# aghasemzadeh/OpenMPL

Measured on AMD Instinct MI355X. Metric: poses/sec (V=4, J=17, batch=1024 per GPU) fp32, higher is better.
Workload: dtype f32; 1 GPU; Human3.6M config: V=4 J=17 batch=1024 fp32, CHOSEN flag set, depth 12, DIM 32, heads 8; global_batch=1024, parallelism=single GPU

## Files before the change

openmpl_amd/csrc/spt_packed.hip:

```cpp
#include "spt_pack.hpp"
#include "spt_stage.hpp"

namespace mpl {

constexpr int ATS = 36;
constexpr int HS = 68;
constexpr int KV_F = SJ * SH * SEQ * 4;
constexpr int SPT3_RING_BYTES = (ROWS * XS + 2 * KV_F + ROWS * ATS) * 4;
constexpr int SPT3_LDS_BYTES = 160 * 1024;
constexpr int SPT3_HID_OFF = 3072;
constexpr int SPT3_Q_OFF = 20480;
static_assert(SPT3_HID_OFF + ROWS * HS <= 2 * KV_F + ROWS * ATS, "HID does not fit its alias");
static_assert((SPT3_HID_OFF + ROWS * HS - 2 * KV_F) * 4 <= SPT3_Q_OFF, "HID reaches into the staged qkv weights");
static_assert(SPT3_Q_OFF + 12 * 1024 <= ROWS * ATS * 4, "staged qkv weights do not fit behind HID in ATT");
static_assert(SPT3_RING_BYTES + 8 * 1024 + 2 * SPT3_NPAR * 4 <= SPT3_LDS_BYTES, "spare LDS too small");

typedef float f32x2 __attribute__((ext_vector_type(2)));

__device__ inline float spt_window_scale(float v) {
    if (!(v > 0.f) || !(v < 3.0e38f)) return 1.0f;
    int e;
    (void)frexpf(32768.0f / v, &e);
    e = e - 1 < -100 ? -100 : (e - 1 > 100 ? 100 : e - 1);
    return ldexpf(1.0f, e);
}

__global__ __launch_bounds__(256) void spt_pack_kernel(const float* __restrict__ qkv_w, const float* __restrict__ qkv_b,
                                                        const float* __restrict__ ln1_w, const float* __restrict__ ln1_b,
                                                        const float* __restrict__ proj_w, const float* __restrict__ proj_b,
                                                        const float* __restrict__ fc1_w, const float* __restrict__ fc1_b,
                                                        const float* __restrict__ ln2_w, const float* __restrict__ ln2_b,
                                                        const float* __restrict__ fc2_w, const float* __restrict__ fc2_b,
                                                        char* __restrict__ dst, int fold_q) {
    __shared__ float Wf[8192];
    __shared__ float cn[SPT_NCOL], sw[SPT_NCOL], bnd[SPT_NCOL], scal[2];
    const int tid = threadIdx.x;
    for (int i = tid; i < 8192; i += 256) {
        float w;
        if (i < 3072) w = qkv_w[i] * ln1_w[i & 31];
        else if (i < 4096) w = proj_w[i - 3072];
        else if (i < 6144) w = fc1_w[i - 4096] * ln2_w[i & 31];
        else w = fc2_w[i - 6144];
        Wf[i] = w;
    }
    __syncthreads();
    if (tid < SPT_NCOL) {
        const int n = tid;
        const float *wr, *raw, *beta = nullptr;
        int K = 32;
        float bias;
        if (n < 96) { wr = Wf + n * 32; raw = qkv_w + n * 32; beta = ln1_b; bias = qkv_b[n]; }
        else if (n < 128) { wr = Wf + 3072 + (n - 96) * 32; raw = proj_w + (n - 96) * 32; bias = proj_b[n - 96]; }
        else if (n < 192) { wr = Wf + 4096 + (n - 128) * 32; raw = fc1_w + (n - 128) * 32; beta = ln2_b; bias = fc1_b[n - 128]; }
        else { wr = Wf + 6144 + (n - 192) * 64; raw = fc2_w + (n - 192) * 64; bias = fc2_b[n - 192]; K = 64; }
        float amax = 0.f;
        double ss = 0.0, c = (double)bias;
        for (int k = 0; k < K; ++k) {
            amax = fmaxf(amax, fabsf(wr[k]));
            ss += (double)wr[k] * (double)wr[k];
            if (beta) c += (double)raw[k] * (double)beta[k];
        }
        float s = 1.0f;
        if (amax > 0.f && amax < 3.0e38f) {
            int e;
            (void)frexpf(amax, &e);
            e = 14 - e;
            e = e < -100 ? -100 : (e > 100 ? 100 : e);
            s = ldexpf(1.0f, e);
        }
        cn[n] = (float)c;
        sw[n] = s;
        bnd[n] = beta ? (float)(sqrt(32.0) * sqrt(ss)) + fabsf((float)c) : 0.f;
    }
    __syncthreads();
    if (tid == 0) {
        float batt = 0.f, bhid = 0.f;
        for (int n = 64; n < 96; ++n) batt = fmaxf(batt, bnd[n]);
        for (int n = SPT_C_FC1; n < SPT_C_FC2; ++n) bhid = fmaxf(bhid, bnd[n]);
        scal[0] = spt_window_scale(batt);
        scal[1] = spt_window_scale(bhid);
    }
    __syncthreads();
    float* vec = reinterpret_cast<float*>(dst + SPT_PACK_VEC);
    if (tid < SPT_NCOL) {
        const int n = tid;
        float c = cn[n], sc;
        if (n < 96) sc = 1.0f / (SPT_SA * sw[n]);
        else if (n < 128) sc = 1.0f / (scal[0] * sw[n]);
        else if (n < 192) sc = 1.0f / (SPT_SA * sw[n]);
        else sc = 1.0f / (scal[1] * sw[n]);
        if (n < 32 && fold_q) { c *= SPT_QS; sc *= SPT_QS; }
        vec[n] = c;
        vec[SPT_NCOL + n] = sc;
    }
    if (tid < 8) vec[2 * SPT_NCOL + tid] = tid == 0 ? scal[0] : (tid == 1 ? 0.5f * scal[1] : 0.f);
    sf16x8* frag = reinterpret_cast<sf16x8*>(dst);
    for (int idx = tid; idx < 16 * 64; idx += 256) {
        const int lane = idx & 63, u = idx >> 6, li = lane & 15, kq = lane >> 4;
        const float* src;
        int n;
        if (u < 6) { n = 16 * u + li; src = Wf + n * 32 + 8 * kq; }
        else if (u < 8) { n = 16 * (u - 6) + li; src = Wf + 3072 + n * 32 + 8 * kq; n += SPT_C_PROJ; }
        else if (u < 12) { n = 16 * (u - 8) + li; src = Wf + 4096 + n * 32 + 8 * kq; n += SPT_C_FC1; }
        else { n = 16 * ((u - 12) >> 1) + li; src = Wf + 6144 + n * 64 + 32 * ((u - 12) & 1) + 8 * kq; n += SPT_C_FC2; }
        float x[8];
#pragma unroll
        for (int j = 0; j < 8; ++j) x[j] = src[j] * sw[n];
        sf16x8 hi, lo;
        spt_split2(x, hi, lo);
        frag[(size_t)(u * 2) * 64 + lane] = hi;
        frag[(size_t)(u * 2 + 1) * 64 + lane] = lo;
    }
}

int launch_spt_pack(const mpl_block_weights* bw_host, unsigned short* dst, int fold_q, hipStream_t s) {
    const mpl_block_weights* b = bw_host;
    if (!b || !dst || !b->qkv_w || !b->proj_w || !b->fc1_w || !b->fc2_w || !b->qkv_b || !b->proj_b || !b->fc1_b || !b->fc2_b ||
        !b->ln1_w || !b->ln1_b || !b->ln2_w || !b->ln2_b)
        return MPL_E_INVALID;
    ProfScope prof(MPL_K_PACK, s);
    hipLaunchKernelGGL(spt_pack_kernel, dim3(1), dim3(256), 0, s, b->qkv_w, b->qkv_b, b->ln1_w, b->ln1_b, b->proj_w, b->proj_b, b->fc1_w,
                       b->fc1_b, b->ln2_w, b->ln2_b, b->fc2_w, b->fc2_b, reinterpret_cast<char*>(dst), fold_q);
    return hip_check_launch();
}

size_t spt_pack_bytes() { return SPT_PACK_BYTES; }

template <int SS>
__global__ __launch_bounds__(NTHR, 1) void spt3_kernel(const SptParams p) {
    constexpr int RLIVE = SJ * SS;
    constexpr int MTS = (RLIVE + 15) / 16;
    constexpr int NT = (MTS + 3) / 4;
    extern __shared__ __attribute__((aligned(16))) float smem[];
    float* X = smem;
    float* Kb = smem + ROWS * XS;
    float* Vb = Kb + KV_F;
    float* ATT = Vb + KV_F;
    float* HID = Kb + SPT3_HID_OFF;
    char* S_W = reinterpret_cast<char*>(ATT + ROWS * ATS);
    float* S_PAR = reinterpret_cast<float*>(S_W + 8 * 1024);
    char* R_F1 = reinterpret_cast<char*>(Kb);
    char* R_Q = reinterpret_cast<char*>(ATT) + SPT3_Q_OFF;

    const int tid = threadIdx.x, lane = tid & 63;
    const int wave = __builtin_amdgcn_readfirstlane(tid >> 6);
    const int li = lane & 15, kq = lane >> 4;
    auto phase_sync = [&]() {
        asm volatile("s_waitcnt vmcnt(0)" ::: "memory");
        __syncthreads();
    };
    const int hg = wave & 1, part = wave >> 1;
    const int view = blockIdx.x % p.V;
    const int b0 = (blockIdx.x / p.V) * SS;
    const int sl = li % SS;
    const mpl_spt_set set = p.sets[(p.flags & MPL_F_MULTI_SPT) ? view : 0];
    const float* pose = p.poses[view];
    const float* ray = p.rays[view];
    const float* cen = p.centers[view];

    auto stage_w = [&](char* dst, const unsigned short* pack, int byte_off, int n_pieces) {
        const unsigned l0 = (unsigned)(uintptr_t)(__attribute__((address_space(3))) char*)dst;
        for (int i = wave; i < n_pieces; i += NWAVE)
            ::mpl::dma16(reinterpret_cast<const float*>(reinterpret_cast<const char*>(pack) + byte_off + i * 1024) + lane * 4,
                         l0 + (unsigned)(i * 1024));
    };
    auto load_par = [&](const mpl_block_weights& b) -> float4 {
        if (tid >= SPT3_NPAR / 4) return float4{0.f, 0.f, 0.f, 0.f};
        return ld4(G(reinterpret_cast<const float*>(reinterpret_cast<const char*>(b.qkv_w3) + SPT_PACK_VEC)) + 4 * tid);
    };
    auto store_par = [&](int app_of, const float4& v) {
        if (tid < SPT3_NPAR / 4) st4(S_PAR + (app_of & 1) * SPT3_NPAR + 4 * tid, v);
    };
    mpl_block_weights bw;
    if (p.n_apps > 0) {
        bw = set.blocks[p.sched[0] & 0x7f];
        stage_w(R_Q, bw.qkv_w3, SPT_PACK_QKV, 12);
    }
    const float4 par0 = p.n_apps > 0 ? load_par(bw) : float4{0.f, 0.f, 0.f, 0.f};
    spt_embed<true, SS>(p, set, X, tid, b0, pose, ray, cen, SS, MTS * 16);
    store_par(0, par0);
    phase_sync();

    auto load_w = [&](const char* region, int unit, sf16x8 (&w)[2]) { spt_load_unit(region, unit, lane, w); };
    auto ln_frag = [&](int m, sf16x8& ah, sf16x8& al) {
        const float* xr = X + (m * 16 + li) * XS + 8 * kq;
        spt_ln_split(::mpl::ld4(xr), ::mpl::ld4(xr + 4), ah, al);
    };
    auto raw_frag = [&](const float* rowp, sf16x8& ah, sf16x8& al) {
        const float4 x0 = ::mpl::ld4(rowp), x1 = ::mpl::ld4(rowp + 4);
        const float y[8] = {x0.x, x0.y, x0.z, x0.w, x1.x, x1.y, x1.z, x1.w};
        spt_split2(y, ah, al);
    };

    for (int app = 0; app < p.n_apps; ++app) {
        const bool weighted = (p.sched[app] & 0x80) != 0;
        bw = set.blocks[p.sched[app] & 0x7f];
        const unsigned short* pack = bw.qkv_w3;
        const float* par = S_PAR + (app & 1) * SPT3_NPAR;
        stage_w(S_W, pack, SPT_PACK_PROJ, 4);
        {
            sf16x8 wq[3][2];
            float4 bq[3], sq[3];
#pragma unroll
            for (int c = 0; c < 3; ++c) {
                load_w(R_Q, 2 * c + hg, wq[c]);
                bq[c] = ::mpl::ld4(par + SPT_C_QKV + 32 * c + 16 * hg + 4 * kq);
                sq[c] = ::mpl::ld4(par + SPT_NCOL + SPT_C_QKV + 32 * c + 16 * hg + 4 * kq);
            }
            float4 q[NT];
#pragma unroll
            for (int t = 0; t < NT; ++t) {
                q[t] = float4{0.f, 0.f, 0.f, 0.f};
                if (part + 4 * t < MTS && !(p.abl & 8)) {
                    const int m = part + 4 * t;
                    const int j = (16 * m + li) / SS;
                    const bool live = 16 * m + li < RLIVE;
                    sf16x8 ah, al;
                    ln_frag(m, ah, al);
                    const f32x4 z = {0.f, 0.f, 0.f, 0.f};
                    const f32x4 cq = mfma3(wq[0], ah, al, z), ck = mfma3(wq[1], ah, al, z), cv = mfma3(wq[2], ah, al, z);
                    q[t] = float4{fmaf(cq[0], sq[0].x, bq[0].x), fmaf(cq[1], sq[0].y, bq[0].y), fmaf(cq[2], sq[0].z, bq[0].z),
                                  fmaf(cq[3], sq[0].w, bq[0].w)};
                    const int h = 4 * hg + kq;
                    const float kx = fmaf(ck[0], sq[1].x, bq[1].x), ky = fmaf(ck[1], sq[1].y, bq[1].y);
                    const float kz = fmaf(ck[2], sq[1].z, bq[1].z), kw = fmaf(ck[3], sq[1].w, bq[1].w);
                    if (live && j < SJ - 1) {
                        float* kp = Kb + ((((j >> 1) * 2) * SH + h) * SS + sl) * 4 + (j & 1);
                        kp[0] = kx;
                        kp[2] = ky;
                        kp[SH * SS * 4] = kz;
                        kp[SH * SS * 4 + 2] = kw;
                    } else if (live) {
                        st4(Kb + (SJ - 1) * SH * SS * 4 + (h * SS + sl) * 4, float4{kx, ky, kz, kw});
                    }
                    if (live)
                        st4(Vb + ((j * SH + h) * SS + sl) * 4, float4{fmaf(cv[0], sq[2].x, bq[2].x), fmaf(cv[1], sq[2].y, bq[2].y),
                                                                       fmaf(cv[2], sq[2].z, bq[2].z), fmaf(cv[3], sq[2].w, bq[2].w)});
                }
            }
            phase_sync();
            if (!(p.abl & 1)) {
                const int h = 4 * hg + kq;
                float sc[NT][SJ];
#pragma unroll
                for (int jp = 0; jp < SJ / 2; ++jp) {
                    const float4 k01 = ::mpl::ld4(Kb + (((jp * 2) * SH + h) * SS + sl) * 4);
                    const float4 k23 = ::mpl::ld4(Kb + (((jp * 2 + 1) * SH + h) * SS + sl) * 4);
                    const f32x2 kx = {k01.x, k01.y}, ky = {k01.z, k01.w}, kz = {k23.x, k23.y}, kw = {k23.z, k23.w};
#pragma unroll
                    for (int t = 0; t < NT; ++t) {
                        const f32x2 qx = {q[t].x, q[t].x}, qy = {q[t].y, q[t].y}, qz = {q[t].z, q[t].z}, qw = {q[t].w, q[t].w};
                        f32x2 s2 = qx * kx;
                        s2 = __builtin_elementwise_fma(qy, ky, s2);
                        s2 = __builtin_elementwise_fma(qz, kz, s2);
                        s2 = __builtin_elementwise_fma(qw, kw, s2);
                        sc[t][2 * jp] = s2[0];
                        sc[t][2 * jp + 1] = s2[1];
                    }
                }
                {
                    const float4 k = ::mpl::ld4(Kb + (SJ - 1) * SH * SS * 4 + (h * SS + sl) * 4);
#pragma unroll
                    for (int t = 0; t < NT; ++t)
                        sc[t][SJ - 1] = fmaf(q[t].w, k.w, fmaf(q[t].z, k.z, fmaf(q[t].y, k.y, q[t].x * k.x)));
                }
                const float s_att = par[2 * SPT_NCOL];
                float inv[NT];
#pragma unroll
                for (int t = 0; t < NT; ++t) {
                    float mx = sc[t][0];
#pragma unroll
                    for (int j = 1; j < SJ; ++j) mx = fmaxf(mx, sc[t][j]);
                    float l = 0.f;
#pragma unroll
                    for (int j = 0; j < SJ; ++j) {
                        sc[t][j] = __builtin_amdgcn_exp2f(sc[t][j] - mx);
                        l += sc[t][j];
                    }
                    inv[t] = __builtin_amdgcn_rcpf(l) * s_att;
                    if (weighted) {
                        const int b = b0 + sl, r = 16 * (part + 4 * t) + li;
                        inv[t] *= (b < p.B && r < RLIVE) ? pose[((size_t)b * SJ + r / SS) * 3 + 2] : 0.f;
                    }
                }
                float4 o[NT];
#pragma unroll
                for (int t = 0; t < NT; ++t) o[t] = float4{0.f, 0.f, 0.f, 0.f};
#pragma unroll
                for (int j = 0; j < SJ; ++j) {
                    const float4 v = ::mpl::ld4(Vb + ((j * SH + h) * SS + sl) * 4);
#pragma unroll
                    for (int t = 0; t < NT; ++t) {
                        const float pj = sc[t][j];
                        o[t].x = fmaf(pj, v.x, o[t].x);
                        o[t].y = fmaf(pj, v.y, o[t].y);
                        o[t].z = fmaf(pj, v.z, o[t].z);
                        o[t].w = fmaf(pj, v.w, o[t].w);
                    }
                }
#pragma unroll
                for (int t = 0; t < NT; ++t) {
                    o[t] = float4{o[t].x * inv[t], o[t].y * inv[t], o[t].z * inv[t], o[t].w * inv[t]};
                    if (weighted) {
                        const float big = fmaxf(fmaxf(fabsf(o[t].x), fabsf(o[t].y)), fmaxf(fabsf(o[t].z), fabsf(o[t].w)));
                        if (!(big <= 65000.f)) {
                            const float qn = __builtin_nanf("");
                            o[t] = float4{qn, qn, qn, qn};
                            if (p.err_host) __hip_atomic_fetch_or(p.err_host, 2u, __ATOMIC_RELAXED, __HIP_MEMORY_SCOPE_SYSTEM);
                        }
                    }
                }
#pragma unroll
                for (int t = 0; t < NT; ++t)
                    if (part + 4 * t < MTS) st4(ATT + ((part + 4 * t) * 16 + li) * ATS + 4 * h, o[t]);
            }
        }
        phase_sync();
        {
            stage_w(R_F1, pack, SPT_PACK_FC1, 8);
            sf16x8 wp[2][2];
            float4 bp[2], sp[2];
#pragma unroll
            for (int n = 0; n < 2; ++n) {
                load_w(S_W, n, wp[n]);
                bp[n] = ::mpl::ld4(par + SPT_C_PROJ + 16 * n + 4 * kq);
                sp[n] = ::mpl::ld4(par + SPT_NCOL + SPT_C_PROJ + 16 * n + 4 * kq);
            }
            const int lo = (MTS * 2 * wave) / NWAVE, hi = (MTS * 2 * (wave + 1)) / NWAVE;
            for (int m = lo >> 1; m <= ((hi - 1) >> 1) && !(p.abl & 32); ++m) {
                sf16x8 ah, al;
                raw_frag(ATT + (m * 16 + li) * ATS + 8 * kq, ah, al);
#pragma unroll
                for (int n = 0; n < 2; ++n) {
                    const int u = 2 * m + n;
                    if (u < lo || u >= hi) continue;
                    const f32x4 c = mfma3(wp[n], ah, al, f32x4{0.f, 0.f, 0.f, 0.f});
                    float* xd = X + (m * 16 + li) * XS + 16 * n + 4 * kq;
                    const float4 x = ::mpl::ld4(xd);
                    st4(xd, float4{x.x + fmaf(c[0], sp[n].x, bp[n].x), x.y + fmaf(c[1], sp[n].y, bp[n].y),
                                   x.z + fmaf(c[2], sp[n].z, bp[n].z), x.w + fmaf(c[3], sp[n].w, bp[n].w)});
                }
            }
        }
        phase_sync();
        {
            stage_w(S_W, pack, SPT_PACK_FC2, 8);
            sf16x8 w1[4][2];
            float4 b1[4], s1[4];
#pragma unroll
            for (int n = 0; n < 4; ++n) {
                load_w(R_F1, n, w1[n]);
                b1[n] = ::mpl::ld4(par + SPT_C_FC1 + 16 * n + 4 * kq);
                s1[n] = ::mpl::ld4(par + SPT_NCOL + SPT_C_FC1 + 16 * n + 4 * kq);
            }
            const float hs = par[2 * SPT_NCOL + 1];
            const int lo = (MTS * 4 * wave) / NWAVE, hi = (MTS * 4 * (wave + 1)) / NWAVE;
            for (int m = lo >> 2; m <= ((hi - 1) >> 2) && !(p.abl & 64); ++m) {
                sf16x8 ah, al;
                ln_frag(m, ah, al);
#pragma unroll
                for (int n = 0; n < 4; ++n) {
                    const int u = 4 * m + n;
                    if (u < lo || u >= hi) continue;
                    const f32x4 c = mfma3(w1[n], ah, al, f32x4{0.f, 0.f, 0.f, 0.f});
                    st4(HID + (m * 16 + li) * HS + 16 * n + 4 * kq,
                        float4{gelu_as_scaled(fmaf(c[0], s1[n].x, b1[n].x), hs), gelu_as_scaled(fmaf(c[1], s1[n].y, b1[n].y), hs),
                               gelu_as_scaled(fmaf(c[2], s1[n].z, b1[n].z), hs), gelu_as_scaled(fmaf(c[3], s1[n].w, b1[n].w), hs)});
                }
            }
        }
        phase_sync();
        {
            float4 parn = float4{0.f, 0.f, 0.f, 0.f};
            if (app + 1 < p.n_apps) {
                const mpl_block_weights bn = set.blocks[p.sched[app + 1] & 0x7f];
                stage_w(R_Q, bn.qkv_w3, SPT_PACK_QKV, 12);
                parn = load_par(bn);
            }
            sf16x8 w2[2][2][2];
            float4 b2[2], s2[2];
#pragma unroll
            for (int n = 0; n < 2; ++n) {
                load_w(S_W, 2 * n, w2[n][0]);
                load_w(S_W, 2 * n + 1, w2[n][1]);
                b2[n] = ::mpl::ld4(par + SPT_C_FC2 + 16 * n + 4 * kq);
                s2[n] = ::mpl::ld4(par + SPT_NCOL + SPT_C_FC2 + 16 * n + 4 * kq);
            }
            const int lo = (MTS * 2 * wave) / NWAVE, hi = (MTS * 2 * (wave + 1)) / NWAVE;
            for (int m = lo >> 1; m <= ((hi - 1) >> 1) && !(p.abl & 128); ++m) {
                sf16x8 ah0, al0, ah1, al1;
                raw_frag(HID + (m * 16 + li) * HS + 8 * kq, ah0, al0);
                raw_frag(HID + (m * 16 + li) * HS + 32 + 8 * kq, ah1, al1);
#pragma unroll
                for (int n = 0; n < 2; ++n) {
                    const int u = 2 * m + n;
                    if (u < lo || u >= hi) continue;
                    f32x4 c = mfma3(w2[n][0], ah0, al0, f32x4{0.f, 0.f, 0.f, 0.f});
                    c = mfma3(w2[n][1], ah1, al1, c);
                    float* xd = X + (m * 16 + li) * XS + 16 * n + 4 * kq;
                    const float4 x = ::mpl::ld4(xd);
                    st4(xd, float4{x.x + fmaf(c[0], s2[n].x, b2[n].x), x.y + fmaf(c[1], s2[n].y, b2[n].y),
                                   x.z + fmaf(c[2], s2[n].z, b2[n].z), x.w + fmaf(c[3], s2[n].w, b2[n].w)});
                }
            }
            if (app + 1 < p.n_apps) store_par(app + 1, parn);
        }
        phase_sync();
    }
    spt_epilogue<true, SS>(p, X, tid, view, b0, pose, ray, cen, SS, MTS * 16);
}

template <int SS>
static int launch_spt3(const SptParams& p, int grid, hipStream_t s) {
    if (int rc = kernel_lds_once<spt3_kernel<SS>>(SPT3_LDS_BYTES)) return rc;
    hipLaunchKernelGGL(spt3_kernel<SS>, dim3(grid), dim3(NTHR), SPT3_LDS_BYTES, s, p);
    return hip_check_launch();
}

int launch_spt_packed(const SptParams& p, int ss, int grid, hipStream_t s) {
    switch (ss) {
        case 1: return launch_spt3<1>(p, grid, s);
        case 2: return launch_spt3<2>(p, grid, s);
        case 4: return launch_spt3<4>(p, grid, s);
        case 8: return launch_spt3<8>(p, grid, s);
        case 16: return launch_spt3<16>(p, grid, s);
        default: return MPL_E_INVALID;
    }
}

}
```

openmpl_amd/csrc/spt_stage.hpp:

```cpp
#pragma once
#include "common.hpp"

namespace mpl {

constexpr int SJ = 17;
constexpr int SD = 32;
constexpr int SH = 8;
constexpr int SEQ = 16;
constexpr int ROWS = SEQ * SJ;
constexpr int XS = 36;
constexpr int NTHR = 512;
constexpr int NWAVE = NTHR / 64;
constexpr int SPT_SMALL_SPW = 8;

struct SptParams {
    const float* poses[MPL_MAX_VIEWS];
    const float* rays[MPL_MAX_VIEWS];
    const float* centers[MPL_MAX_VIEWS];
    const mpl_spt_set* sets;
    const float *snorm_w, *snorm_b;
    const float *pos3d_embed, *pos3d_view, *pos3d_lin_w, *pos3d_lin_b;
    const float *ray_w, *ray_b, *cfpt_w, *cfpt_b;
    float* xs;
    int B, V, in_ch, n_apps;
    unsigned flags;
    int c3;
    int spw;
    int abl;
    unsigned* err_host;
    unsigned char sched[MPL_MAX_APPS];
};

int launch_spt_native(const SptParams& p, int form, int grid, hipStream_t s);
int launch_spt_packed(const SptParams& p, int ss, int grid, hipStream_t s);

typedef const __attribute__((address_space(1))) float* gfp;
__device__ __forceinline__ gfp G(const float* p) { return (gfp)p; }
__device__ __forceinline__ float4 ld4(gfp p) {
    typedef float v4 __attribute__((ext_vector_type(4)));
    const v4 t = *reinterpret_cast<const __attribute__((address_space(1))) v4*>(p);
    return make_float4(t.x, t.y, t.z, t.w);
}

template <bool TM, int SS = SEQ>
__device__ __forceinline__ void row_to_sj(int r, int& sq, int& j) {
    if (TM) { j = r / SS; sq = r % SS; }
    else { sq = r / SJ; j = r - sq * SJ; }
}

template <bool TM, int SS = SEQ>
__device__ __forceinline__ void spt_embed(const SptParams& p, const mpl_spt_set& set, float* X, int tid, int b0,
                                          const float* pose, const float* ray, const float* cen, int nseq = SEQ, int nrows = ROWS) {
    for (int idx = tid; idx < nrows * SD; idx += NTHR) {
        const int r = idx >> 5, c = idx & 31;
        int sq, j;
        row_to_sj<TM, SS>(r, sq, j);
        const int b = b0 + sq;
        float x = 0.f;
        if (b < p.B && sq < nseq && j < SJ) {
            const float* in = pose + ((size_t)b * SJ + j) * 3;
            const float* we = set.embed_w + c * p.in_ch;
            x = set.embed_b[c] + we[0] * in[0] + we[1] * in[1];
            if (p.in_ch == 3) x += we[2] * in[2];
            if (p.flags & MPL_F_CONF_ADD) x += set.conf_w[c] * in[2] + set.conf_b[c];
            if (p.flags & MPL_F_CONF_MULT) x *= set.conf_w[c] * in[2] + set.conf_b[c];
            x += set.pos_embed[j * SD + c];
            if (p.flags & MPL_F_POS3D_SPATIAL) {
                if (p.flags & MPL_F_POS3D_LEARN) {
                    x += p.pos3d_embed[j * p.c3 + c];
                } else {
                    const float* rr = ray + ((size_t)b * SJ + j) * 3;
                    const float* cc = cen + (size_t)b * 3;
                    const float vx = rr[0] - cc[0], vy = rr[1] - cc[1], vz = rr[2] - cc[2];
                    const float nrm = fmaxf(sqrtf(vx * vx + vy * vy + vz * vz), 1e-12f);
                    const float* wl = p.pos3d_lin_w + c * 3;
                    x += p.pos3d_lin_b[c] + wl[0] * (vx / nrm) + wl[1] * (vy / nrm) + wl[2] * (vz / nrm);
                }
            }
        }
        X[r * XS + c] = x;
    }
}

template <bool TM, int SS = SEQ>
__device__ __forceinline__ void spt_epilogue(const SptParams& p, const float* X, int tid, int view, int b0, const float* pose,
                                             const float* ray, const float* cen, int nseq = SEQ, int nrows = ROWS) {
    const bool to_rays = (p.flags & MPL_F_POS3D_TO_RAYS) && (p.flags & MPL_F_RAYS_TOKEN);
    const bool ray_tok = !(p.flags & MPL_F_POS3D_TO_RAYS) && (p.flags & MPL_F_RAYS_TOKEN);
    const int cw = to_rays ? 2 * SD : SD;
    const int Df = SJ * SD * ((p.flags & MPL_F_RAYS_TOKEN) ? 2 : 1);
    for (int r = tid; r < nrows; r += NTHR) {
        int sq, j;
        row_to_sj<TM, SS>(r, sq, j);
        const int b = b0 + sq;
        if (b >= p.B || sq >= nseq || j >= SJ) continue;
        const float* xr = X + r * XS;
        float v[SD];
        float s = 0.f;
#pragma unroll
        for (int c = 0; c < SD; c += 4) {
            const float4 t = ld4(xr + c);
            v[c] = t.x; v[c + 1] = t.y; v[c + 2] = t.z; v[c + 3] = t.w;
            s += (t.x + t.y) + (t.z + t.w);
        }
        const float mean = s * (1.0f / 32.0f);
        float ss = 0.f;
#pragma unroll
        for (int c = 0; c < SD; ++c) {
            v[c] -= mean;
            ss = fmaf(v[c], v[c], ss);
        }
        const float rstd = 1.0f / sqrtf(ss * (1.0f / 32.0f) + 1e-6f);
        const float conf = pose[((size_t)b * SJ + j) * 3 + 2];
        float dx = 0.f, dy = 0.f, dz = 0.f, nx = 0.f, ny = 0.f, nz = 0.f;
        const bool need_dir = (p.flags & MPL_F_RAYS_TOKEN) ||
                              (!(p.flags & MPL_F_POS3D_SPATIAL) && !(p.flags & MPL_F_POS3D_LEARN));
        if (need_dir) {
            const float* rr = ray + ((size_t)b * SJ + j) * 3;
            const float* cc = cen + (size_t)b * 3;
            dx = rr[0] - cc[0]; dy = rr[1] - cc[1]; dz = rr[2] - cc[2];
            const float nrm = fmaxf(sqrtf(dx * dx + dy * dy + dz * dz), 1e-12f);
            nx = dx / nrm; ny = dy / nrm; nz = dz / nrm;
        }
        auto pos3d = [=](int c) -> float {
            if (p.flags & MPL_F_POS3D_SPATIAL) return p.pos3d_view[j * p.c3 + c];
            if (p.flags & MPL_F_POS3D_LEARN) return p.pos3d_embed[j * p.c3 + c];
            const float* wl = p.pos3d_lin_w + c * 3;
            return p.pos3d_lin_b[c] + wl[0] * nx + wl[1] * ny + wl[2] * nz;
        };
        auto ray_emb = [=](int c) -> float {
            const float* wr = p.ray_w + c * 3;
            return p.ray_b[c] + wr[0] * dx + wr[1] * dy + wr[2] * dz;
        };
        float* orow = p.xs + ((size_t)b * p.V + view) * Df;
        float* o1 = orow + j * cw;
#pragma unroll
        for (int c = 0; c < SD; c += 4) {
            float t[4];
#pragma unroll
            for (int q = 0; q < 4; ++q) {
                float y = v[c + q] * rstd * p.snorm_w[c + q] + p.snorm_b[c + q];
                if (p.flags & MPL_F_CONF_IN_FPT) y += p.cfpt_w[c + q] * conf + p.cfpt_b[c + q];
                t[q] = y + pos3d(c + q);
            }
            st4(o1 + c, float4{t[0], t[1], t[2], t[3]});
        }
        if (to_rays) {
#pragma unroll
            for (int c = 0; c < SD; c += 4) {
                float t[4];
#pragma unroll
                for (int q = 0; q < 4; ++q) t[q] = ray_emb(c + q) + pos3d(SD + c + q);
                st4(o1 + SD + c, float4{t[0], t[1], t[2], t[3]});
            }
        } else if (ray_tok) {
            float* o2 = orow + (SJ + j) * SD;
#pragma unroll
            for (int c = 0; c < SD; c += 4) st4(o2 + c, float4{ray_emb(c), ray_emb(c + 1), ray_emb(c + 2), ray_emb(c + 3)});
        }
    }
}

}
```

Before: 830,000 poses/s.

## Templatize spt3 kernel on wave count and split attention into full and tail tiles

The spt3 kernel now takes the wave count as a template parameter and launches 16 waves for larger sequence tiles, 8 otherwise, spreading row tiles across more waves. Attention is restructured into a lambda run separately for full tiles and one ragged tail tile, which avoids per-tile bounds checks. Scores and outputs are held as packed f32x2 so packed FMA can be used. The aim is more parallelism per block and less divergence and register pressure in attention, at the cost of more threads sharing the same LDS and barriers.

Measured after the change: 831,500 poses/s (median of 3 runs). No clear change (+0.2%).

```diff
diff --git a/openmpl_amd/csrc/spt_packed.hip b/openmpl_amd/csrc/spt_packed.hip
--- a/openmpl_amd/csrc/spt_packed.hip
+++ b/openmpl_amd/csrc/spt_packed.hip
@@ -126,11 +126,13 @@
 
 size_t spt_pack_bytes() { return SPT_PACK_BYTES; }
 
-template <int SS>
-__global__ __launch_bounds__(NTHR, 1) void spt3_kernel(const SptParams p) {
+template <int SS, int NW>
+__global__ __launch_bounds__(NW * 64, 1) void spt3_kernel(const SptParams p) {
     constexpr int RLIVE = SJ * SS;
     constexpr int MTS = (RLIVE + 15) / 16;
-    constexpr int NT = (MTS + 3) / 4;
+    constexpr int NWQ = NW / 2;
+    constexpr int NT = (MTS + NWQ - 1) / NWQ;
+    constexpr int NTF = MTS / NWQ;
     extern __shared__ __attribute__((aligned(16))) float smem[];
     float* X = smem;
     float* Kb = smem + ROWS * XS;
@@ -142,17 +144,25 @@
     char* R_F1 = reinterpret_cast<char*>(Kb);
     char* R_Q = reinterpret_cast<char*>(ATT) + SPT3_Q_OFF;
 
-    const int tid = threadIdx.x, lane = tid & 63;
+    const int tid = threadIdx.x;
+    int lane = tid & 63;
     const int wave = __builtin_amdgcn_readfirstlane(tid >> 6);
-    const int li = lane & 15, kq = lane >> 4;
+    int li = lane & 15, kq = lane >> 4;
     auto phase_sync = [&]() {
         asm volatile("s_waitcnt vmcnt(0)" ::: "memory");
         __syncthreads();
     };
     const int hg = wave & 1, part = wave >> 1;
+    auto has_tile = [&](int t) { return t < NTF || part + NWQ * t < MTS; };
     const int view = blockIdx.x % p.V;
     const int b0 = (blockIdx.x / p.V) * SS;
-    const int sl = li % SS;
+    int sl = li % SS;
+    auto relane = [&]() {
+        asm volatile("" : "+v"(lane));
+        li = lane & 15;
+        kq = lane >> 4;
+        sl = li % SS;
+    };
     const mpl_spt_set set = p.sets[(p.flags & MPL_F_MULTI_SPT) ? view : 0];
     const float* pose = p.poses[view];
     const float* ray = p.rays[view];
@@ -160,7 +170,7 @@
 
     auto stage_w = [&](char* dst, const unsigned short* pack, int byte_off, int n_pieces) {
         const unsigned l0 = (unsigned)(uintptr_t)(__attribute__((address_space(3))) char*)dst;
-        for (int i = wave; i < n_pieces; i += NWAVE)
+        for (int i = wave; i < n_pieces; i += NW)
             ::mpl::dma16(reinterpret_cast<const float*>(reinterpret_cast<const char*>(pack) + byte_off + i * 1024) + lane * 4,
                          l0 + (unsigned)(i * 1024));
     };
@@ -177,7 +187,7 @@
         stage_w(R_Q, bw.qkv_w3, SPT_PACK_QKV, 12);
     }
     const float4 par0 = p.n_apps > 0 ? load_par(bw) : float4{0.f, 0.f, 0.f, 0.f};
-    spt_embed<true, SS>(p, set, X, tid, b0, pose, ray, cen, SS, MTS * 16);
+    spt_embed<true, SS, NW * 64>(p, set, X, tid, b0, pose, ray, cen, SS, MTS * 16);
     store_par(0, par0);
     phase_sync();
 
@@ -197,6 +207,7 @@
         bw = set.blocks[p.sched[app] & 0x7f];
         const unsigned short* pack = bw.qkv_w3;
         const float* par = S_PAR + (app & 1) * SPT3_NPAR;
+        relane();
         stage_w(S_W, pack, SPT_PACK_PROJ, 4);
         {
             sf16x8 wq[3][2];
@@ -211,8 +222,8 @@
 #pragma unroll
             for (int t = 0; t < NT; ++t) {
                 q[t] = float4{0.f, 0.f, 0.f, 0.f};
-                if (part + 4 * t < MTS && !(p.abl & 8)) {
-                    const int m = part + 4 * t;
+                if (has_tile(t) && !(p.abl & 8)) {
+                    const int m = part + NWQ * t;
                     const int j = (16 * m + li) / SS;
                     const bool live = 16 * m + li < RLIVE;
                     sf16x8 ah, al;
@@ -239,68 +250,80 @@
                 }
             }
             phase_sync();
-            if (!(p.abl & 1)) {
+            auto attend = [&](auto t0_c, auto n_c) {
+                constexpr int T0 = decltype(t0_c)::value, N = decltype(n_c)::value;
                 const int h = 4 * hg + kq;
-                float sc[NT][SJ];
+                f32x2 sc[N][SJ / 2];
+                float sl_[N];
 #pragma unroll
                 for (int jp = 0; jp < SJ / 2; ++jp) {
                     const float4 k01 = ::mpl::ld4(Kb + (((jp * 2) * SH + h) * SS + sl) * 4);
                     const float4 k23 = ::mpl::ld4(Kb + (((jp * 2 + 1) * SH + h) * SS + sl) * 4);
                     const f32x2 kx = {k01.x, k01.y}, ky = {k01.z, k01.w}, kz = {k23.x, k23.y}, kw = {k23.z, k23.w};
 #pragma unroll
-                    for (int t = 0; t < NT; ++t) {
-                        const f32x2 qx = {q[t].x, q[t].x}, qy = {q[t].y, q[t].y}, qz = {q[t].z, q[t].z}, qw = {q[t].w, q[t].w};
+                    for (int t = 0; t < N; ++t) {
+                        const float4 qt = q[T0 + t];
+                        const f32x2 qx = {qt.x, qt.x}, qy = {qt.y, qt.y}, qz = {qt.z, qt.z}, qw = {qt.w, qt.w};
                         f32x2 s2 = qx * kx;
                         s2 = __builtin_elementwise_fma(qy, ky, s2);
                         s2 = __builtin_elementwise_fma(qz, kz, s2);
                         s2 = __builtin_elementwise_fma(qw, kw, s2);
-                        sc[t][2 * jp] = s2[0];
-                        sc[t][2 * jp + 1] = s2[1];
+                        sc[t][jp] = s2;
                     }
                 }
                 {
                     const float4 k = ::mpl::ld4(Kb + (SJ - 1) * SH * SS * 4 + (h * SS + sl) * 4);
 #pragma unroll
-                    for (int t = 0; t < NT; ++t)
-                        sc[t][SJ - 1] = fmaf(q[t].w, k.w, fmaf(q[t].z, k.z, fmaf(q[t].y, k.y, q[t].x * k.x)));
+                    for (int t = 0; t < N; ++t) {
+                        const float4 qt = q[T0 + t];
+                        sl_[t] = fmaf(qt.w, k.w, fmaf(qt.z, k.z, fmaf(qt.y, k.y, qt.x * k.x)));
+                    }
                 }
                 const float s_att = par[2 * SPT_NCOL];
-                float inv[NT];
-#pragma unroll
-                for (int t = 0; t < NT; ++t) {
-                    float mx = sc[t][0];
-#pragma unroll
-                    for (int j = 1; j < SJ; ++j) mx = fmaxf(mx, sc[t][j]);
+                float inv[N];
+#pragma unroll
+                for (int t = 0; t < N; ++t) {
+                    float mx = sc[t][0][0];
+#pragma unroll
+                    for (int j = 1; j < SJ - 1; ++j) mx = fmaxf(mx, sc[t][j >> 1][j & 1]);
+                    mx = fmaxf(mx, sl_[t]);
                     float l = 0.f;
 #pragma unroll
-                    for (int j = 0; j < SJ; ++j) {
-                        sc[t][j] = __builtin_amdgcn_exp2f(sc[t][j] - mx);
-                        l += sc[t][j];
-                    }
+                    for (int j = 0; j < SJ - 1; ++j) {
+                        sc[t][j >> 1][j & 1] = __builtin_amdgcn_exp2f(sc[t][j >> 1][j & 1] - mx);
+                        l += sc[t][j >> 1][j & 1];
+                    }
+                    sl_[t] = __builtin_amdgcn_exp2f(sl_[t] - mx);
+                    l += sl_[t];
+#pragma unroll
+                    for (int jp = 0; jp < SJ / 2; ++jp) asm volatile("" : "+v"(sc[t][jp]));
                     inv[t] = __builtin_amdgcn_rcpf(l) * s_att;
                     if (weighted) {
-                        const int b = b0 + sl, r = 16 * (part + 4 * t) + li;
+                        const int b = b0 + sl, r = 16 * (part + NWQ * (T0 + t)) + li;
                         inv[t] *= (b < p.B && r < RLIVE) ? pose[((size_t)b * SJ + r / SS) * 3 + 2] : 0.f;
                     }
                 }
-                float4 o[NT];
-#pragma unroll
-                for (int t = 0; t < NT; ++t) o[t] = float4{0.f, 0.f, 0.f, 0.f};
+                f32x2 oxy[N], ozw[N];
+#pragma unroll
+                for (int t = 0; t < N; ++t) oxy[t] = ozw[t] = f32x2{0.f, 0.f};
 #pragma unroll
                 for (int j = 0; j < SJ; ++j) {
                     const float4 v = ::mpl::ld4(Vb + ((j * SH + h) * SS + sl) * 4);
-#pragma unroll
-                    for (int t = 0; t < NT; ++t) {
-                        const float pj = sc[t][j];
-                        o[t].x = fmaf(pj, v.x, o[t].x);
-                        o[t].y = fmaf(pj, v.y, o[t].y);
-                        o[t].z = fmaf(pj, v.z, o[t].z);
-                        o[t].w = fmaf(pj, v.w, o[t].w);
-                    }
-                }
-#pragma unroll
-                for (int t = 0; t < NT; ++t) {
-                    o[t] = float4{o[t].x * inv[t], o[t].y * inv[t], o[t].z * inv[t], o[t].w * inv[t]};
+                    const f32x2 vxy = {v.x, v.y}, vzw = {v.z, v.w};
+#pragma unroll
+                    for (int t = 0; t < N; ++t) {
+                        f32x2 pj;
+                        if (j == SJ - 1) pj = f32x2{sl_[t], sl_[t]};
+                        else if (j & 1) pj = __builtin_shufflevector(sc[t][j >> 1], sc[t][j >> 1], 1, 1);
+                        else pj = __builtin_shufflevector(sc[t][j >> 1], sc[t][j >> 1], 0, 0);
+                        oxy[t] = __builtin_elementwise_fma(pj, vxy, oxy[t]);
+                        ozw[t] = __builtin_elementwise_fma(pj, vzw, ozw[t]);
+                    }
+                }
+                float4 o[N];
+#pragma unroll
+                for (int t = 0; t < N; ++t) {
+                    o[t] = float4{oxy[t][0] * inv[t], oxy[t][1] * inv[t], ozw[t][0] * inv[t], ozw[t][1] * inv[t]};
                     if (weighted) {
                         const float big = fmaxf(fmaxf(fabsf(o[t].x), fabsf(o[t].y)), fmaxf(fabsf(o[t].z), fabsf(o[t].w)));
                         if (!(big <= 65000.f)) {
@@ -311,8 +334,12 @@
                     }
                 }
 #pragma unroll
-                for (int t = 0; t < NT; ++t)
-                    if (part + 4 * t < MTS) st4(ATT + ((part + 4 * t) * 16 + li) * ATS + 4 * h, o[t]);
+                for (int t = 0; t < N; ++t) st4(ATT + ((part + NWQ * (T0 + t)) * 16 + li) * ATS + 4 * h, o[t]);
+            };
+            if (!(p.abl & 1)) {
+                if constexpr (NT > NTF)
+                    if (has_tile(NTF)) attend(std::integral_constant<int, NTF>{}, std::integral_constant<int, 1>{});
+                if constexpr (NTF > 0) attend(std::integral_constant<int, 0>{}, std::integral_constant<int, NTF>{});
             }
         }
         phase_sync();
@@ -326,7 +353,7 @@
                 bp[n] = ::mpl::ld4(par + SPT_C_PROJ + 16 * n + 4 * kq);
                 sp[n] = ::mpl::ld4(par + SPT_NCOL + SPT_C_PROJ + 16 * n + 4 * kq);
             }
-            const int lo = (MTS * 2 * wave) / NWAVE, hi = (MTS * 2 * (wave + 1)) / NWAVE;
+            const int lo = (MTS * 2 * wave) / NW, hi = (MTS * 2 * (wave + 1)) / NW;
             for (int m = lo >> 1; m <= ((hi - 1) >> 1) && !(p.abl & 32); ++m) {
                 sf16x8 ah, al;
                 raw_frag(ATT + (m * 16 + li) * ATS + 8 * kq, ah, al);
@@ -354,7 +381,7 @@
                 s1[n] = ::mpl::ld4(par + SPT_NCOL + SPT_C_FC1 + 16 * n + 4 * kq);
             }
             const float hs = par[2 * SPT_NCOL + 1];
-            const int lo = (MTS * 4 * wave) / NWAVE, hi = (MTS * 4 * (wave + 1)) / NWAVE;
+            const int lo = (MTS * 4 * wave) / NW, hi = (MTS * 4 * (wave + 1)) / NW;
             for (int m = lo >> 2; m <= ((hi - 1) >> 2) && !(p.abl & 64); ++m) {
                 sf16x8 ah, al;
                 ln_frag(m, ah, al);
@@ -386,7 +413,7 @@
                 b2[n] = ::mpl::ld4(par + SPT_C_FC2 + 16 * n + 4 * kq);
                 s2[n] = ::mpl::ld4(par + SPT_NCOL + SPT_C_FC2 + 16 * n + 4 * kq);
             }
-            const int lo = (MTS * 2 * wave) / NWAVE, hi = (MTS * 2 * (wave + 1)) / NWAVE;
+            const int lo = (MTS * 2 * wave) / NW, hi = (MTS * 2 * (wave + 1)) / NW;
             for (int m = lo >> 1; m <= ((hi - 1) >> 1) && !(p.abl & 128); ++m) {
                 sf16x8 ah0, al0, ah1, al1;
                 raw_frag(HID + (m * 16 + li) * HS + 8 * kq, ah0, al0);
@@ -407,13 +434,17 @@
         }
         phase_sync();
     }
-    spt_epilogue<true, SS>(p, X, tid, view, b0, pose, ray, cen, SS, MTS * 16);
-}
+    spt_epilogue<true, SS, NW * 64>(p, X, tid, view, b0, pose, ray, cen, SS, MTS * 16);
+}
+
+template <int SS>
+constexpr int SPT3_WAVES = SS >= 16 ? 16 : 8;
 
 template <int SS>
 static int launch_spt3(const SptParams& p, int grid, hipStream_t s) {
-    if (int rc = kernel_lds_once<spt3_kernel<SS>>(SPT3_LDS_BYTES)) return rc;
-    hipLaunchKernelGGL(spt3_kernel<SS>, dim3(grid), dim3(NTHR), SPT3_LDS_BYTES, s, p);
+    constexpr int NW = SPT3_WAVES<SS>;
+    if (int rc = kernel_lds_once<spt3_kernel<SS, NW>>(SPT3_LDS_BYTES)) return rc;
+    hipLaunchKernelGGL((spt3_kernel<SS, NW>), dim3(grid), dim3(NW * 64), SPT3_LDS_BYTES, s, p);
     return hip_check_launch();
 }
 
diff --git a/openmpl_amd/csrc/spt_stage.hpp b/openmpl_amd/csrc/spt_stage.hpp
--- a/openmpl_amd/csrc/spt_stage.hpp
+++ b/openmpl_amd/csrc/spt_stage.hpp
@@ -48,10 +48,10 @@
     else { sq = r / SJ; j = r - sq * SJ; }
 }
 
-template <bool TM, int SS = SEQ>
+template <bool TM, int SS = SEQ, int NTH = NTHR>
 __device__ __forceinline__ void spt_embed(const SptParams& p, const mpl_spt_set& set, float* X, int tid, int b0,
                                           const float* pose, const float* ray, const float* cen, int nseq = SEQ, int nrows = ROWS) {
-    for (int idx = tid; idx < nrows * SD; idx += NTHR) {
+    for (int idx = tid; idx < nrows * SD; idx += NTH) {
         const int r = idx >> 5, c = idx & 31;
         int sq, j;
         row_to_sj<TM, SS>(r, sq, j);
@@ -82,14 +82,14 @@
     }
 }
 
-template <bool TM, int SS = SEQ>
+template <bool TM, int SS = SEQ, int NTH = NTHR>
 __device__ __forceinline__ void spt_epilogue(const SptParams& p, const float* X, int tid, int view, int b0, const float* pose,
                                              const float* ray, const float* cen, int nseq = SEQ, int nrows = ROWS) {
     const bool to_rays = (p.flags & MPL_F_POS3D_TO_RAYS) && (p.flags & MPL_F_RAYS_TOKEN);
     const bool ray_tok = !(p.flags & MPL_F_POS3D_TO_RAYS) && (p.flags & MPL_F_RAYS_TOKEN);
     const int cw = to_rays ? 2 * SD : SD;
     const int Df = SJ * SD * ((p.flags & MPL_F_RAYS_TOKEN) ? 2 : 1);
-    for (int r = tid; r < nrows; r += NTHR) {
+    for (int r = tid; r < nrows; r += NTH) {
         int sq, j;
         row_to_sj<TM, SS>(r, sq, j);
         const int b = b0 + sq;
```
